# scroll-tech/zkevm-circuits

Measured on NVIDIA H100. Metric: SuperCircuit-shaped k=20 create_proof seconds (halo2 KZG/SHPLONK, Blake2b transcript), lower is better.
Workload: dtype u256 (8x u32 Montgomery limbs, BN254 Fr/Fq)

## Files before the change

zkevm-circuits_b200/csrc/common.cuh:

```cuda
#pragma once
#include <cuda_runtime.h>
#include <stdint.h>
#include <stdio.h>
#include <map>
#include <string>
#include <vector>
#include <array>
#include "../../include/zkb200.h"
#include "ff.cuh"
#include "g1.cuh"

namespace zkb {

void set_error(const char *fmt, ...);

#define ZKB_CUDA(expr)                                                                                   \
    do {                                                                                                 \
        cudaError_t _e = (expr);                                                                         \
        if (_e != cudaSuccess) {                                                                         \
            zkb::set_error("%s:%d %s -> %s", __FILE__, __LINE__, #expr, cudaGetErrorString(_e));         \
            return _e == cudaErrorMemoryAllocation ? ZKB_ERR_ALLOC : ZKB_ERR_CUDA;                       \
        }                                                                                                \
    } while (0)

#define ZKB_TRY(expr)                    \
    do {                                 \
        int32_t _r = (expr);             \
        if (_r != ZKB_OK) return _r;     \
    } while (0)

#define ZKB_ARG(cond)                                                            \
    do {                                                                         \
        if (!(cond)) {                                                           \
            zkb::set_error("%s:%d invalid argument: %s", __FILE__, __LINE__, #cond); \
            return ZKB_ERR_ARG;                                                  \
        }                                                                        \
    } while (0)

struct NttPlan {
    uint32_t log_n = 0;
    int npass = 0;
    int bits[3] = {0, 0, 0};
    Fr *tw_lo = nullptr;
    Fr *tw_hi = nullptr;
    Fr *loc[3] = {nullptr, nullptr, nullptr};
    Fr *tw_b[2] = {nullptr, nullptr};
    Fr *tw_b_scaled = nullptr;
    Fr scaled_key;
    bool has_scaled = false;
};

struct DeviceBuffer {
    void *ptr = nullptr;
    size_t bytes = 0;
};

}

struct zkb_ctx {
    int device = 0;
    cudaStream_t stream = nullptr;
    cudaStream_t copy_stream = nullptr;
    int sm_count = 132;
    size_t mem_bytes = 0;
    void *nccl_comm = nullptr;
    int rank = 0, nranks = 1;
    void *win_local = nullptr;
    size_t win_bytes = 0;
    void *win_peers[16] = {nullptr};
    std::map<std::array<uint64_t, 6>, void *> shard_tw;
    uint64_t launches = 0;
    bool prof_on = false;
    struct ProfPair { cudaEvent_t a, b; int cls; };
    std::vector<ProfPair> prof_pending;
    std::vector<cudaEvent_t> prof_free;
    double prof_ms[8] = {};
    uint64_t prof_count[8] = {};
    bool ntt_ready = false;
    uint64_t msm_last_adds = 0;
    uint32_t msm_last_levels = 0;
    std::map<std::array<uint64_t, 5>, zkb::NttPlan> ntt_plans;
    zkb::DeviceBuffer scratch[14];
    std::multimap<size_t, void *> block_cache;
    size_t block_cache_bytes = 0;
    void *pinned = nullptr;
    size_t pinned_bytes = 0;
};

struct zkb_srs {
    zkb_ctx *ctx = nullptr;
    uint32_t k = 0;
    uint64_t n = 0;
    zkb::G1Affine *g = nullptr, *g_lagrange = nullptr;
    zkb::G1Affine *g_shift = nullptr, *g_lagrange_shift = nullptr;
    std::vector<std::pair<void *, size_t>> blocks;
};

namespace zkb {
int32_t scratch_get(zkb_ctx *ctx, int slot, size_t bytes, void **out);
int32_t block_alloc(zkb_ctx *ctx, size_t bytes, void **out, size_t *got);
void block_free(zkb_ctx *ctx, void *p, size_t bytes);
inline cudaStream_t pick_stream(zkb_ctx *ctx, void *stream) { return stream ? (cudaStream_t)stream : ctx->stream; }
enum ProfClass { PROF_NTT = 0, PROF_MSM_ACC = 1, PROF_EXPR = 2, PROF_OTHER = 3, PROF_CHECK_GATES = 4, PROF_CHECK_LOOKUPS = 5,
                 PROF_CHECK_COPIES = 6, PROF_CHECK_EXTRACT = 7, PROF_CLASSES = 8 };
struct ProfScope {
    zkb_ctx *ctx;
    cudaStream_t st;
    cudaEvent_t a = nullptr, b = nullptr;
    int cls;
    ProfScope(zkb_ctx *c, int cl, cudaStream_t s) : ctx(c), st(s), cls(cl) {
        if (!ctx->prof_on) return;
        auto get = [&]() { cudaEvent_t e = nullptr; if (!ctx->prof_free.empty()) { e = ctx->prof_free.back(); ctx->prof_free.pop_back(); } else cudaEventCreate(&e); return e; };
        a = get(); b = get();
        cudaEventRecord(a, st);
    }
    ~ProfScope() {
        if (!a) return;
        cudaEventRecord(b, st);
        ctx->prof_pending.push_back({a, b, cls});
    }
};

Fr host_root_of_unity(uint32_t k);
Fr host_zeta();
int32_t ntt_fr_device(zkb_ctx *ctx, const Fr *src, Fr *dst, uint32_t log_n, const Fr &omega, const Fr *scale_host, int coset_zeta,
                      const Fr *d_in_scale, cudaStream_t st);
int32_t ntt_fr_batch_device(zkb_ctx *ctx, const Fr *const *h_src, Fr *const *h_dst, uint32_t count, uint32_t log_n,
                            const Fr &omega, const Fr *scale_host, int coset_zeta, const Fr *d_in_scale, cudaStream_t st);
struct NttPeerRoute {
    const Fr *out_tw;
    bool routed;
    uint32_t log_blk, rank;
    int nranks;
    Fr *peers[16];
};
int32_t ntt_fr_batch_device_ex(zkb_ctx *ctx, const Fr *const *h_src, Fr *const *h_dst, uint32_t count, uint32_t log_n, const Fr &omega,
                               const Fr *scale_host, int coset_zeta, const Fr *d_in_scale, const NttPeerRoute *route, cudaStream_t st);
int32_t msm_g1_device(zkb_ctx *ctx, const Fr *scalars, const G1Affine *bases, uint64_t n, G1Affine *out_affine_host, cudaStream_t st);
uint32_t msm_max_batch(uint64_t n);
uint32_t msm_shift_copies(uint64_t n);
int32_t msm_build_shifted_bases(zkb_ctx *ctx, const G1Affine *bases, uint64_t n, G1Affine *out, cudaStream_t st);
int32_t msm_g1_batch_device_ex(zkb_ctx *ctx, const Fr *const *d_scalar_cols, uint32_t batch, const G1Affine *bases, uint64_t n,
                               G1Affine *out_affine_host, bool shifted, cudaStream_t st);
int32_t msm_g1_batch_device(zkb_ctx *ctx, const Fr *const *d_scalar_cols, uint32_t batch, const G1Affine *bases, uint64_t n,
                            G1Affine *out_affine_host, cudaStream_t st);
int32_t srs_create(zkb_ctx *ctx, uint32_t k, const G1Affine *g, bool g_on_device, const G1Affine *g_lagrange, bool gl_on_device, zkb_srs **out);
int32_t srs_commit_many(zkb_srs *s, int basis, const Fr *const *cols, uint32_t count, uint64_t len, G1Affine *out_host, cudaStream_t st);
int32_t fr_powers_device(zkb_ctx *ctx, const Fr &base, uint64_t n, Fr *out, cudaStream_t st);
int32_t poly_eval_device(zkb_ctx *ctx, const Fr *const *d_polys, uint32_t num, uint64_t n, const Fr &x, Fr *out_host, cudaStream_t st);
int32_t prefix_product_device(zkb_ctx *ctx, const Fr *in, uint64_t n, const Fr &init, Fr *out, cudaStream_t st);
int32_t prefix_sum_device(zkb_ctx *ctx, const Fr *in, uint64_t n, const Fr &init, Fr *out, cudaStream_t st);
int32_t kate_division_device(zkb_ctx *ctx, const Fr *a, uint64_t n, const Fr &u, Fr *q, cudaStream_t st);
int32_t lincomb_device(zkb_ctx *ctx, const Fr *const *d_polys, const Fr *d_coefs, uint32_t num, uint64_t n, Fr *out, bool accumulate, cudaStream_t st);
int32_t batch_invert_device(zkb_ctx *ctx, const Fr *a, Fr *out, uint64_t n, cudaStream_t st);
int32_t comm_allreduce_u64(zkb_ctx *ctx, void *dev_buf, size_t count, cudaStream_t st);
int32_t comm_allgather(zkb_ctx *ctx, const void *send, void *recv, size_t bytes_per_rank, cudaStream_t st);
int32_t comm_alltoall(zkb_ctx *ctx, const void *send, void *recv, size_t bytes_per_block, cudaStream_t st);
int32_t comm_barrier(zkb_ctx *ctx, cudaStream_t st);
int32_t comm_window(zkb_ctx *ctx, size_t bytes, cudaStream_t st);

struct DevPool {
    zkb_ctx *ctx = nullptr;
    std::vector<std::pair<void *, size_t>> ptrs;
    ~DevPool() {
        if (!ctx) return;
        cudaStreamSynchronize(ctx->stream);
        for (auto &p : ptrs) block_free(ctx, p.first, p.second);
    }
    int32_t alloc(size_t bytes, void **out) {
        size_t got = 0;
        ZKB_TRY(block_alloc(ctx, bytes ? bytes : 32, out, &got));
        ptrs.push_back({*out, got});
        return ZKB_OK;
    }
    int32_t fr(uint64_t n, Fr **out) { return alloc(n * sizeof(Fr), (void **)out); }
};

enum ScratchSlot { SCR_NTT = 0, SCR_MSM_A = 1, SCR_MSM_B = 2, SCR_MSM_C = 3, SCR_HOSTIO_A = 4, SCR_HOSTIO_B = 5, SCR_MISC = 6, SCR_MISC2 = 7, SCR_MSM_TBL = 8, SCR_COMM = 9, SCR_NTT_DESC = 10, SCR_MSM_D = 11, SCR_COMM_FLAG = 12, SCR_SHARD = 13 };
}
```

zkevm-circuits_b200/csrc/msm.cu:

```cuda
#include "common.cuh"
#include <string.h>
#include <algorithm>

namespace zkb {

struct MsmCfg {
    uint32_t c;
    uint32_t windows;
    uint32_t half;
    uint32_t seg_log;
    uint32_t shifted;
    uint32_t n32;
};

static MsmCfg choose_cfg(uint64_t n) {
    uint32_t lg = 0;
    while ((1ull << (lg + 1)) <= n) ++lg;
    int c = (int)lg - 4;
    if (c < 3) c = 3;
    if (c > 20) c = 20;
    MsmCfg m;
    m.c = (uint32_t)c;
    m.windows = (255 + m.c - 1) / m.c;
    m.half = 1u << (m.c - 1);
    m.seg_log = 0;
    m.shifted = 0;
    m.n32 = 0;
    return m;
}

__device__ __forceinline__ uint32_t raw_window(const uint32_t s[8], uint32_t bit, uint32_t c) {
    const uint32_t limb = bit >> 5, off = bit & 31;
    uint64_t v = s[limb];
    if (limb + 1 < 8) v |= (uint64_t)s[limb + 1] << 32;
    return (uint32_t)(v >> off) & ((1u << c) - 1);
}

template <int MODE>
__global__ void msm_digits_kernel(const Fr *const *__restrict__ scalar_cols, uint64_t n, MsmCfg m, uint32_t *__restrict__ counts,
                                  uint32_t *__restrict__ cursors, uint32_t *__restrict__ sorted) {
    const uint64_t i = blockIdx.x * (uint64_t)blockDim.x + threadIdx.x;
    if (i >= n) return;
    const uint32_t col_base = blockIdx.y * (m.shifted ? m.half : m.windows * m.half);
    const Fr s = fp_to_canonical(fp_load(scalar_cols[blockIdx.y] + i));
    uint32_t carry = 0;
    for (uint32_t w = 0; w < m.windows; ++w) {
        const uint32_t bit = w * m.c;
        uint32_t d = (bit < 256 ? raw_window(s.l, bit, m.c) : 0) + carry;
        uint32_t neg = 0;
        if (d > m.half) { d = (1u << m.c) - d; neg = 1; carry = 1; }
        else carry = 0;
        if (d != 0) {
            const uint32_t b = col_base + (m.shifted ? 0u : w * m.half) + (d - 1);
            if (MODE == 0) atomicAdd(&counts[b], 1u);
            else {
                const uint32_t pos = atomicAdd(&cursors[b], 1u);
                sorted[pos] = ((uint32_t)i + (m.shifted ? w * m.n32 : 0u)) | (neg << 31);
            }
        }
    }
}

constexpr int SCAN_T = 512, SCAN_PER = 4, SCAN_BLK = SCAN_T * SCAN_PER;

__device__ __forceinline__ uint32_t block_exclusive_scan(uint32_t v, uint32_t *total, uint32_t *sm ) {
    const uint32_t lane = threadIdx.x & 31, wid = threadIdx.x >> 5;
    uint32_t x = v;
#pragma unroll
    for (int o = 1; o < 32; o <<= 1) {
        uint32_t y = __shfl_up_sync(0xffffffffu, x, o);
        if (lane >= o) x += y;
    }
    if (lane == 31) sm[wid] = x;
    __syncthreads();
    if (wid == 0) {
        uint32_t t = lane < (blockDim.x >> 5) ? sm[lane] : 0;
#pragma unroll
        for (int o = 1; o < 32; o <<= 1) {
            uint32_t y = __shfl_up_sync(0xffffffffu, t, o);
            if (lane >= o) t += y;
        }
        sm[lane] = t;
    }
    __syncthreads();
    const uint32_t base = wid ? sm[wid - 1] : 0;
    *total = sm[(blockDim.x >> 5) - 1];
    return base + x - v;
}

__global__ void scan_blocks_kernel(const uint32_t *__restrict__ in, uint32_t *__restrict__ out, uint32_t *__restrict__ block_sums, uint64_t n) {
    __shared__ uint32_t sm[32];
    const uint64_t base = (uint64_t)blockIdx.x * SCAN_BLK + (uint64_t)threadIdx.x * SCAN_PER;
    uint32_t v[SCAN_PER], sum = 0;
#pragma unroll
    for (int k = 0; k < SCAN_PER; ++k) { v[k] = base + k < n ? in[base + k] : 0; sum += v[k]; }
    uint32_t total;
    uint32_t ex = block_exclusive_scan(sum, &total, sm);
#pragma unroll
    for (int k = 0; k < SCAN_PER; ++k) { if (base + k < n) out[base + k] = ex; ex += v[k]; }
    if (threadIdx.x == 0) block_sums[blockIdx.x] = total;
}
__global__ void scan_sums_kernel(uint32_t *__restrict__ block_sums, uint32_t nblocks, uint32_t *__restrict__ grand_total) {
    __shared__ uint32_t sm[32];
    uint32_t running = 0;
    for (uint32_t s = 0; s < nblocks; s += SCAN_T) {
        const uint32_t idx = s + threadIdx.x;
        const uint32_t v = idx < nblocks ? block_sums[idx] : 0;
        uint32_t total;
        const uint32_t ex = block_exclusive_scan(v, &total, sm);
        if (idx < nblocks) block_sums[idx] = running + ex;
        running += total;
        __syncthreads();
    }
    if (threadIdx.x == 0 && grand_total) *grand_total = running;
}
__global__ void scan_add_kernel(uint32_t *__restrict__ out, const uint32_t *__restrict__ block_sums, uint64_t n) {
    const uint64_t base = (uint64_t)blockIdx.x * SCAN_BLK + (uint64_t)threadIdx.x * SCAN_PER;
    const uint32_t add = block_sums[blockIdx.x];
#pragma unroll
    for (int k = 0; k < SCAN_PER; ++k)
        if (base + k < n) out[base + k] += add;
}

struct MsmState;
__global__ void scan_blocks_gated_kernel(const uint32_t *__restrict__ in, uint32_t *const outs0, uint32_t *const outs1, const uint32_t *st_words,
                                         uint32_t *__restrict__ block_sums, uint64_t n) {
    if (st_words[0] <= 1) return;
    uint32_t *out = st_words[1] ? outs0 : outs1;
    __shared__ uint32_t sm[32];
    const uint64_t base = (uint64_t)blockIdx.x * SCAN_BLK + (uint64_t)threadIdx.x * SCAN_PER;
    uint32_t v[SCAN_PER], sum = 0;
#pragma unroll
    for (int k = 0; k < SCAN_PER; ++k) { v[k] = base + k < n ? in[base + k] : 0; sum += v[k]; }
    uint32_t total;
    uint32_t ex = block_exclusive_scan(sum, &total, sm);
#pragma unroll
    for (int k = 0; k < SCAN_PER; ++k) { if (base + k < n) out[base + k] = ex; ex += v[k]; }
    if (threadIdx.x == 0) block_sums[blockIdx.x] = total;
}
__global__ void scan_sums_gated_kernel(uint32_t *__restrict__ block_sums, uint32_t nblocks, uint32_t *const outs0, uint32_t *const outs1,
                                       const uint32_t *st_words, uint64_t n) {
    if (st_words[0] <= 1) return;
    uint32_t *out = st_words[1] ? outs0 : outs1;
    __shared__ uint32_t sm[32];
    uint32_t running = 0;
    for (uint32_t s = 0; s < nblocks; s += SCAN_T) {
        const uint32_t idx = s + threadIdx.x;
        const uint32_t v = idx < nblocks ? block_sums[idx] : 0;
        uint32_t total;
        const uint32_t ex = block_exclusive_scan(v, &total, sm);
        if (idx < nblocks) block_sums[idx] = running + ex;
        running += total;
        __syncthreads();
    }
    if (threadIdx.x == 0) out[n] = running;
}
__global__ void scan_add_gated_kernel(uint32_t *const outs0, uint32_t *const outs1, const uint32_t *st_words, const uint32_t *__restrict__ block_sums,
                                      uint64_t n) {
    if (st_words[0] <= 1) return;
    uint32_t *out = st_words[1] ? outs0 : outs1;
    const uint64_t base = (uint64_t)blockIdx.x * SCAN_BLK + (uint64_t)threadIdx.x * SCAN_PER;
    const uint32_t add = block_sums[blockIdx.x];
#pragma unroll
    for (int k = 0; k < SCAN_PER; ++k)
        if (base + k < n) out[base + k] += add;
}

static void exclusive_scan_u32(zkb_ctx *ctx, const uint32_t *in, uint32_t *out, uint64_t n, uint32_t *tmp, cudaStream_t st) {
    const uint32_t nblocks = (uint32_t)((n + SCAN_BLK - 1) / SCAN_BLK);
    scan_blocks_kernel<<<nblocks, SCAN_T, 0, st>>>(in, out, tmp, n);
    scan_sums_kernel<<<1, SCAN_T, 0, st>>>(tmp, nblocks, out + n);
    scan_add_kernel<<<nblocks, SCAN_T, 0, st>>>(out, tmp, n);
    ctx->launches += 3;
}

constexpr uint32_t ACC_CH = 64;
constexpr uint32_t CHUNK = 32;

struct MsmState {
    uint32_t maxlen;
    uint32_t cur;
    uint32_t levels_run;
    uint32_t pad;
    uint64_t extra_adds;
};

__global__ void chunk_count_kernel(const uint32_t *__restrict__ seg_off, uint32_t nseg, uint32_t *__restrict__ tcount, MsmState *st) {
    const uint32_t b = blockIdx.x * blockDim.x + threadIdx.x;
    uint32_t cnt = 0;
    if (b < nseg) {
        const uint32_t lo = seg_off[b], hi = seg_off[b + 1];
        cnt = hi > lo ? (hi - 1) / CHUNK - lo / CHUNK + 1 : 0;
        tcount[b] = cnt;
    }
    for (int o = 16; o > 0; o >>= 1) {
        const uint32_t y = __shfl_down_sync(0xffffffffu, cnt, o);
        cnt = y > cnt ? y : cnt;
    }
    if ((threadIdx.x & 31) == 0 && cnt > 1) atomicMax(&st->maxlen, cnt);
}
__device__ __forceinline__ uint32_t find_segment(const uint32_t *__restrict__ toff, uint32_t nseg, uint32_t t) {
    uint32_t lo = 0, hi = nseg;
    while (hi - lo > 1) {
        const uint32_t mid = (lo + hi) >> 1;
        if (toff[mid] <= t) lo = mid; else hi = mid;
    }
    return lo;
}
__global__ void __launch_bounds__(128) msm_acc_chunk_kernel(const G1Affine *__restrict__ bases, const uint32_t *__restrict__ seg_off,
                                                           const uint32_t *__restrict__ sorted, const uint32_t *__restrict__ toff,
                                                           uint32_t nseg, G1Xyzz *__restrict__ part) {
    const uint32_t total = seg_off[nseg];
    const uint32_t t = blockIdx.x * blockDim.x + threadIdx.x;
    const uint32_t beg = t * CHUNK;
    if (beg >= total) return;
    const uint32_t end = beg + CHUNK < total ? beg + CHUNK : total;
    uint32_t b = find_segment(seg_off, nseg, beg);
    uint32_t b_first = seg_off[b], next = seg_off[b + 1];
    G1Xyzz acc = G1Xyzz::identity();
    uint32_t e = sorted[beg];
    G1Affine p = g1_load_affine(bases + (e & 0x7fffffffu));
    for (uint32_t k = beg; k < end; ++k) {
        if (k == next) {
            g1_store_xyzz(part + toff[b] + (t - b_first / CHUNK), acc);
            acc = G1Xyzz::identity();
            do { ++b; next = seg_off[b + 1]; } while (next <= k);
            b_first = seg_off[b];
        }
        const uint32_t e_cur = e;
        const G1Affine p_cur = p;
        if (k + 1 < end) {
            e = sorted[k + 1];
            p = g1_load_affine(bases + (e & 0x7fffffffu));
        }
        g1_add_mixed(acc, (e_cur >> 31) ? g1_neg(p_cur) : p_cur);
    }
    g1_store_xyzz(part + toff[b] + (t - b_first / CHUNK), acc);
}

struct LevelBufs {
    uint32_t *toff[2];
    G1Xyzz *part[2];
    uint32_t *tcount;
    MsmState *st;
};
__global__ void level_task_count_kernel(LevelBufs L, uint32_t nseg) {
    if (L.st->maxlen <= 1) return;
    const uint32_t *seg_off = L.toff[L.st->cur];
    const uint32_t b = blockIdx.x * blockDim.x + threadIdx.x;
    if (b >= nseg) return;
    const uint32_t len = seg_off[b + 1] - seg_off[b];
    L.tcount[b] = (len + ACC_CH - 1) / ACC_CH;
}
__global__ void __launch_bounds__(128) msm_acc_levelN_kernel(LevelBufs L, uint32_t nseg) {
    if (L.st->maxlen <= 1) return;
    const uint32_t cur = L.st->cur;
    const uint32_t *__restrict__ seg_off = L.toff[cur];
    const uint32_t *__restrict__ toff = L.toff[cur ^ 1];
    const G1Xyzz *__restrict__ in = L.part[cur];
    G1Xyzz *__restrict__ part = L.part[cur ^ 1];
    const uint32_t ntasks = toff[nseg];
    for (uint32_t t = blockIdx.x * blockDim.x + threadIdx.x; t < ntasks; t += gridDim.x * blockDim.x) {
        const uint32_t b = find_segment(toff, nseg, t);
        const uint32_t beg = seg_off[b] + (t - toff[b]) * ACC_CH;
        const uint32_t lim = seg_off[b + 1];
        const uint32_t end = beg + ACC_CH < lim ? beg + ACC_CH : lim;
        G1Xyzz acc = g1_load_xyzz(in + beg);
        for (uint32_t k = beg + 1; k < end; ++k) g1_add(acc, g1_load_xyzz(in + k));
        g1_store_xyzz(part + t, acc);
    }
}
__global__ void level_advance_kernel(LevelBufs L, uint32_t nseg) {
    MsmState *st = L.st;
    if (st->maxlen <= 1) return;
    const uint32_t cur = st->cur;
    st->extra_adds += L.toff[cur][nseg];
    st->maxlen = (st->maxlen + ACC_CH - 1) / ACC_CH;
    st->cur = cur ^ 1;
    st->levels_run++;
}
__global__ void msm_gather_buckets_kernel(LevelBufs L, uint32_t nseg, G1Xyzz *__restrict__ buckets) {
    const uint32_t b = blockIdx.x * blockDim.x + threadIdx.x;
    if (b >= nseg) return;
    const uint32_t cur = L.st->cur;
    const uint32_t *seg_off = L.toff[cur];
    const uint32_t beg = seg_off[b], end = seg_off[b + 1];
    g1_store_xyzz(buckets + b, end > beg ? g1_load_xyzz(L.part[cur] + beg) : G1Xyzz::identity());
}

__global__ void __launch_bounds__(128) msm_wsum_level_kernel(const G1Xyzz *__restrict__ in, uint32_t count, uint32_t log_l, uint32_t windows,
                                                            G1Xyzz *__restrict__ acc_out, G1Xyzz *__restrict__ run_out) {
    const uint32_t L = 1u << log_l;
    const uint32_t segs = (count + L - 1) >> log_l;
    const uint32_t t = blockIdx.x * blockDim.x + threadIdx.x;
    if (t >= windows * segs) return;
    const uint32_t w = t / segs, s = t % segs;
    const uint32_t base = s << log_l;
    const uint32_t len = count - base < L ? count - base : L;
    const G1Xyzz *p = in + (size_t)w * count + base;
    G1Xyzz running = G1Xyzz::identity(), acc = G1Xyzz::identity();
    for (int j = (int)len - 1; j >= 1; --j) {
        g1_add(running, g1_load_xyzz(p + j));
        g1_add(acc, running);
    }
    g1_add(running, g1_load_xyzz(p));
    g1_store_xyzz(acc_out + t, acc);
    g1_store_xyzz(run_out + t, running);
}
__global__ void __launch_bounds__(256) msm_window_sum_kernel(const G1Xyzz *__restrict__ partials, G1Xyzz *__restrict__ window_sums, uint32_t segs) {
    extern __shared__ uint4 sm4[];
    G1Xyzz *sm = reinterpret_cast<G1Xyzz *>(sm4);
    const uint32_t w = blockIdx.x;
    G1Xyzz acc = G1Xyzz::identity();
    for (uint32_t s = threadIdx.x; s < segs; s += blockDim.x) g1_add(acc, g1_load_xyzz(partials + (size_t)w * segs + s));
    sm[threadIdx.x] = acc;
    __syncthreads();
    for (uint32_t o = blockDim.x >> 1; o > 0; o >>= 1) {
        if (threadIdx.x < o) {
            G1Xyzz a = sm[threadIdx.x];
            g1_add(a, sm[threadIdx.x + o]);
            sm[threadIdx.x] = a;
        }
        __syncthreads();
    }
    if (threadIdx.x == 0) g1_store_xyzz(window_sums + w, sm[0]);
}
__global__ void msm_window_combine_kernel(const G1Xyzz *__restrict__ level_sums, const G1Xyzz *__restrict__ all_sum, uint32_t nlevels,
                                          uint32_t log_l, uint32_t windows, G1Xyzz *__restrict__ out) {
    const uint32_t w = blockIdx.x * blockDim.x + threadIdx.x;
    if (w >= windows) return;
    G1Xyzz r = g1_load_xyzz(level_sums + (size_t)(nlevels - 1) * windows + w);
    for (int lv = (int)nlevels - 2; lv >= 0; --lv) {
        for (uint32_t d = 0; d < log_l; ++d) r = g1_dbl(r);
        g1_add(r, g1_load_xyzz(level_sums + (size_t)lv * windows + w));
    }
    g1_add(r, g1_load_xyzz(all_sum + w));
    g1_store_xyzz(out + w, r);
}

__global__ void __launch_bounds__(128) msm_shift_bases_kernel(const G1Affine *__restrict__ in, G1Affine *__restrict__ out, uint64_t n, uint32_t c) {
    const uint64_t i = blockIdx.x * (uint64_t)blockDim.x + threadIdx.x;
    if (i >= n) return;
    G1Xyzz p = G1Xyzz::from_affine(g1_load_affine(in + i));
    for (uint32_t k = 0; k < c; ++k) p = g1_dbl(p);
    g1_store_affine(out + i, g1_to_affine(p));
}

__global__ void __launch_bounds__(128) fixed_base_mul_kernel(G1Affine base, const Fr *__restrict__ scalars, uint64_t n, G1Affine *__restrict__ out) {
    const uint64_t i = blockIdx.x * (uint64_t)blockDim.x + threadIdx.x;
    if (i >= n) return;
    const Fr s = fp_to_canonical(fp_load(scalars + i));
    G1Xyzz acc = G1Xyzz::identity();
    for (int bit = 253; bit >= 0; --bit) {
        acc = g1_dbl(acc);
        if ((s.l[bit >> 5] >> (bit & 31)) & 1) g1_add_mixed(acc, base);
    }
    g1_store_affine(out + i, g1_to_affine(acc));
}

static size_t align_up(size_t v, size_t a) { return (v + a - 1) / a * a; }

uint32_t msm_shift_window_bits(uint64_t n);
uint32_t msm_max_batch(uint64_t n) {
    if (n == 0) return 64;
    const MsmCfg m = choose_cfg(n);
    uint64_t b = (1ull << 28) / (n * m.windows);
    const uint32_t cs = msm_shift_window_bits(n);
    if (cs) {
        const uint64_t bb = (1ull << 31) / ((1ull << (cs - 1)) * 3 * sizeof(G1Xyzz));
        if (bb < b) b = bb;
    }
    if (b < 1) b = 1;
    if (b > 64) b = 64;
    return (uint32_t)b;
}

uint32_t msm_shift_window_bits(uint64_t n) {
    uint32_t lg = 0;
    while ((1ull << (lg + 1)) <= n) ++lg;
    if (lg < 10 || lg > 22) return 0;
    return lg > 20 ? 20 : lg;
}
uint32_t msm_shift_copies(uint64_t n) {
    const uint32_t c = msm_shift_window_bits(n);
    return c ? (255 + c - 1) / c : 0;
}
int32_t msm_build_shifted_bases(zkb_ctx *ctx, const G1Affine *bases, uint64_t n, G1Affine *out, cudaStream_t st) {
    const uint32_t c = msm_shift_window_bits(n), copies = msm_shift_copies(n);
    ZKB_ARG(c != 0);
    ZKB_CUDA(cudaMemcpyAsync(out, bases, n * sizeof(G1Affine), cudaMemcpyDeviceToDevice, st));
    for (uint32_t w = 1; w < copies; ++w) {
        msm_shift_bases_kernel<<<(unsigned)((n + 127) / 128), 128, 0, st>>>(out + (size_t)(w - 1) * n, out + (size_t)w * n, n, c);
        ctx->launches++;
    }
    ZKB_CUDA(cudaGetLastError());
    return ZKB_OK;
}

int32_t msm_g1_batch_device_ex(zkb_ctx *ctx, const Fr *const *d_scalar_cols, uint32_t batch, const G1Affine *bases, uint64_t n,
                               G1Affine *out_affine_host, bool shifted, cudaStream_t st);

int32_t msm_g1_batch_device(zkb_ctx *ctx, const Fr *const *d_scalar_cols, uint32_t batch, const G1Affine *bases, uint64_t n,
                            G1Affine *out_affine_host, cudaStream_t st) {
    return msm_g1_batch_device_ex(ctx, d_scalar_cols, batch, bases, n, out_affine_host, false, st);
}

int32_t msm_g1_batch_device_ex(zkb_ctx *ctx, const Fr *const *d_scalar_cols, uint32_t batch, const G1Affine *bases, uint64_t n,
                               G1Affine *out_affine_host, bool shifted, cudaStream_t st) {
    ZKB_ARG(n < (1ull << 31) && batch >= 1);
    if (n == 0) {
        memset(out_affine_host, 0, sizeof(G1Affine) * batch);
        ctx->msm_last_adds = 0;
        return ZKB_OK;
    }
    MsmCfg m = choose_cfg(n);
    if (shifted) {
        m.c = msm_shift_window_bits(n);
        ZKB_ARG(m.c != 0);
        m.windows = (255 + m.c - 1) / m.c;
        m.half = 1u << (m.c - 1);
        m.shifted = 1;
        m.n32 = (uint32_t)n;
        ZKB_ARG((uint64_t)m.windows * n < (1ull << 31));
    }
    const uint32_t windows1 = m.windows;
    const uint32_t rwin1 = shifted ? 1 : windows1;
    const uint32_t nbuckets = batch * rwin1 * m.half;
    const uint64_t pairs = n * windows1 * batch;
    ZKB_ARG(pairs < (1ull << 32) && (uint64_t)batch * rwin1 * m.half < (1ull << 31));
    uint32_t log_l = 5;
    while (log_l > 3 && (uint64_t)batch * rwin1 * (m.half >> log_l) < 32768) --log_l;

    const size_t cnt_bytes = align_up((size_t)(nbuckets + 2) * 4, 256);
    const size_t tmp_bytes = align_up(((size_t)nbuckets / SCAN_BLK + 2) * 4, 256);
    uint8_t *A = nullptr, *B = nullptr, *C = nullptr;
    ZKB_TRY(scratch_get(ctx, SCR_MSM_A, 6 * cnt_bytes + tmp_bytes + 256, (void **)&A));
    ZKB_TRY(scratch_get(ctx, SCR_MSM_B, pairs * 4, (void **)&B));
    uint32_t *counts = (uint32_t *)A, *offsets = (uint32_t *)(A + cnt_bytes), *cursors = (uint32_t *)(A + 2 * cnt_bytes);
    uint32_t *tcount = (uint32_t *)(A + 3 * cnt_bytes), *toff[2] = {(uint32_t *)(A + 4 * cnt_bytes), (uint32_t *)(A + 5 * cnt_bytes)};
    uint32_t *scan_tmp = (uint32_t *)(A + 6 * cnt_bytes);
    MsmState *d_state = (MsmState *)(A + 6 * cnt_bytes + tmp_bytes);
    uint32_t *sorted = (uint32_t *)B;

    const uint32_t half = m.half;
    const uint32_t wred = rwin1 * batch;
    uint32_t nlevels = 0, cnt = half;
    size_t level_entries = 0;
    while (cnt > 1) { cnt = (cnt + (1u << log_l) - 1) >> log_l; level_entries += 2ull * cnt * wred; nlevels++; }
    if (nlevels == 0) { nlevels = 1; level_entries = 2ull * wred; }
    const size_t part0_n = (size_t)((pairs + CHUNK - 1) / CHUNK) + nbuckets + 1;
    const size_t part1_n = part0_n / ACC_CH + nbuckets + 1;
    ZKB_ARG(part0_n < (1ull << 32));
    const size_t c_entries = part0_n + part1_n + nbuckets + level_entries + (size_t)nlevels * wred + 2ull * wred;
    ZKB_TRY(scratch_get(ctx, SCR_MSM_C, c_entries * sizeof(G1Xyzz), (void **)&C));
    G1Xyzz *part[2] = {(G1Xyzz *)C, (G1Xyzz *)C + part0_n};
    G1Xyzz *buckets = part[1] + part1_n, *lvl = buckets + nbuckets, *lvl_sums = lvl + level_entries, *all_sum = lvl_sums + (size_t)nlevels * wred,
           *wres = all_sum + wred;

    ZKB_CUDA(cudaMemsetAsync(counts, 0, cnt_bytes, st));
    ZKB_CUDA(cudaMemsetAsync(d_state, 0, sizeof(MsmState), st));
    const unsigned tb = 256, bb = (nbuckets + 255) / 256;
    const dim3 gb((unsigned)((n + tb - 1) / tb), batch);
    msm_digits_kernel<0><<<gb, tb, 0, st>>>(d_scalar_cols, n, m, counts, nullptr, nullptr);
    exclusive_scan_u32(ctx, counts, offsets, nbuckets, scan_tmp, st);
    ZKB_CUDA(cudaMemcpyAsync(cursors, offsets, (size_t)nbuckets * 4, cudaMemcpyDeviceToDevice, st));
    msm_digits_kernel<1><<<gb, tb, 0, st>>>(d_scalar_cols, n, m, nullptr, cursors, sorted);
    m.windows = wred;
    chunk_count_kernel<<<bb, 256, 0, st>>>(offsets, nbuckets, tcount, d_state);
    exclusive_scan_u32(ctx, tcount, toff[0], nbuckets, scan_tmp, st);
    {
        const uint64_t max_chunks = (pairs + CHUNK - 1) / CHUNK;
        ProfScope ps_(ctx, PROF_MSM_ACC, st);
        msm_acc_chunk_kernel<<<(unsigned)((max_chunks + 127) / 128), 128, 0, st>>>(bases, offsets, sorted, toff[0], nbuckets, part[0]);
    }
    ctx->launches += 4;
    LevelBufs L;
    L.toff[0] = toff[0]; L.toff[1] = toff[1];
    L.part[0] = part[0]; L.part[1] = part[1];
    L.tcount = tcount;
    L.st = d_state;
    {
        uint64_t bound = (n * (shifted ? windows1 : 1) + CHUNK - 1) / CHUNK + 1;
        const uint32_t nscan = (uint32_t)(((uint64_t)nbuckets + SCAN_BLK - 1) / SCAN_BLK);
        const uint32_t *stw = (const uint32_t *)d_state;
        const unsigned lv_blocks = (unsigned)std::min<uint64_t>((part0_n / ACC_CH + nbuckets + 127) / 128, (uint64_t)ctx->sm_count * 32);
        while (bound > 1) {
            level_task_count_kernel<<<bb, 256, 0, st>>>(L, nbuckets);
            scan_blocks_gated_kernel<<<nscan, SCAN_T, 0, st>>>(tcount, toff[0], toff[1], stw, scan_tmp, nbuckets);
            scan_sums_gated_kernel<<<1, SCAN_T, 0, st>>>(scan_tmp, nscan, toff[0], toff[1], stw, nbuckets);
            scan_add_gated_kernel<<<nscan, SCAN_T, 0, st>>>(toff[0], toff[1], stw, scan_tmp, nbuckets);
            msm_acc_levelN_kernel<<<lv_blocks, 128, 0, st>>>(L, nbuckets);
            level_advance_kernel<<<1, 1, 0, st>>>(L, nbuckets);
            ctx->launches += 6;
            bound = (bound + ACC_CH - 1) / ACC_CH;
        }
    }
    msm_gather_buckets_kernel<<<bb, 256, 0, st>>>(L, nbuckets, buckets);
    ctx->launches++;

    {
        const G1Xyzz *in = buckets;
        uint32_t count = half;
        G1Xyzz *p = lvl;
        for (uint32_t lv = 0; lv < nlevels; ++lv) {
            const uint32_t segs = (count + (1u << log_l) - 1) >> log_l;
            G1Xyzz *acc_out = p, *run_out = p + (size_t)segs * m.windows;
            msm_wsum_level_kernel<<<(m.windows * segs + 127) / 128, 128, 0, st>>>(in, count, log_l, m.windows, acc_out, run_out);
            uint32_t wt = 32;
            while (wt < segs && wt < 256) wt <<= 1;
            msm_window_sum_kernel<<<m.windows, wt, wt * sizeof(G1Xyzz), st>>>(acc_out, lvl_sums + (size_t)lv * m.windows, segs);
            ctx->launches += 2;
            in = run_out;
            count = segs;
            p += 2ull * segs * m.windows;
            if (lv + 1 == nlevels) {
                ZKB_CUDA(cudaMemcpyAsync(all_sum, run_out, (size_t)m.windows * sizeof(G1Xyzz), cudaMemcpyDeviceToDevice, st));
            }
        }
        msm_window_combine_kernel<<<(m.windows + 31) / 32, 32, 0, st>>>(lvl_sums, all_sum, nlevels, log_l, m.windows, wres);
        ctx->launches++;
    }
    ZKB_CUDA(cudaGetLastError());

    std::vector<G1Xyzz> h(m.windows);
    MsmState h_state;
    uint32_t total_pairs = 0;
    ZKB_CUDA(cudaMemcpyAsync(h.data(), wres, m.windows * sizeof(G1Xyzz), cudaMemcpyDeviceToHost, st));
    ZKB_CUDA(cudaMemcpyAsync(&h_state, d_state, sizeof(MsmState), cudaMemcpyDeviceToHost, st));
    ZKB_CUDA(cudaMemcpyAsync(&total_pairs, offsets + nbuckets, 4, cudaMemcpyDeviceToHost, st));
    ZKB_CUDA(cudaStreamSynchronize(st));
    for (uint32_t col = 0; col < batch; ++col) {
        const G1Xyzz *hw = h.data() + (size_t)col * rwin1;
        G1Xyzz acc = hw[rwin1 - 1];
        for (int w = (int)rwin1 - 2; w >= 0; --w) {
            for (uint32_t k = 0; k < m.c; ++k) acc = g1_dbl(acc);
            g1_add(acc, hw[w]);
        }
        out_affine_host[col] = g1_to_affine(acc);
    }
    ctx->msm_last_adds = (uint64_t)total_pairs + h_state.extra_adds + 2ull * nbuckets;
    ctx->msm_last_levels = h_state.levels_run;
    return ZKB_OK;
}

int32_t msm_g1_device(zkb_ctx *ctx, const Fr *scalars, const G1Affine *bases, uint64_t n, G1Affine *out_affine_host, cudaStream_t st) {
    if (n == 0) {
        memset(out_affine_host, 0, sizeof(G1Affine));
        ctx->msm_last_adds = 0;
        return ZKB_OK;
    }
    const Fr **d_tbl = nullptr;
    ZKB_TRY(scratch_get(ctx, SCR_MSM_TBL, 64 * sizeof(Fr *), (void **)&d_tbl));
    ZKB_CUDA(cudaMemcpyAsync(d_tbl, &scalars, sizeof(Fr *), cudaMemcpyHostToDevice, st));
    return msm_g1_batch_device(ctx, d_tbl, 1, bases, n, out_affine_host, st);
}

}
using namespace zkb;

static void emit_outputs(const G1Affine &r, uint64_t out_affine[8], uint64_t *out_jacobian, uint8_t *out_compressed) {
    memcpy(out_affine, &r, 64);
    if (out_jacobian) {
        memcpy(out_jacobian, &r, 64);
        Fq z = r.is_identity() ? Fq::zero() : Fq::one();
        memcpy(out_jacobian + 8, &z, 32);
    }
    if (out_compressed) g1_compress(r, out_compressed);
}

extern "C" int32_t zkb_msm_g1_dev(zkb_ctx *ctx, const uint64_t *scalars_dev, const uint64_t *bases_dev, uint64_t n, uint64_t out_affine[8],
                                  uint64_t *out_jacobian, uint8_t *out_compressed, void *stream) {
    ZKB_ARG(ctx && out_affine && (n == 0 || (scalars_dev && bases_dev)));
    ZKB_CUDA(cudaSetDevice(ctx->device));
    G1Affine r;
    ZKB_TRY(msm_g1_device(ctx, (const Fr *)scalars_dev, (const G1Affine *)bases_dev, n, &r, pick_stream(ctx, stream)));
    emit_outputs(r, out_affine, out_jacobian, out_compressed);
    return ZKB_OK;
}

extern "C" int32_t zkb_msm_g1_host(zkb_ctx *ctx, const uint64_t *scalars_host, const uint64_t *bases_host, uint64_t n, uint64_t out_affine[8],
                                   uint64_t *out_jacobian, uint8_t *out_compressed) {
    ZKB_ARG(ctx && out_affine && (n == 0 || (scalars_host && bases_host)));
    ZKB_CUDA(cudaSetDevice(ctx->device));
    void *ds = nullptr, *db = nullptr;
    if (n) {
        ZKB_TRY(scratch_get(ctx, SCR_HOSTIO_A, n * 32, &ds));
        ZKB_TRY(scratch_get(ctx, SCR_HOSTIO_B, n * 64, &db));
        ZKB_CUDA(cudaMemcpyAsync(ds, scalars_host, n * 32, cudaMemcpyHostToDevice, ctx->stream));
        ZKB_CUDA(cudaMemcpyAsync(db, bases_host, n * 64, cudaMemcpyHostToDevice, ctx->stream));
    }
    return zkb_msm_g1_dev(ctx, (const uint64_t *)ds, (const uint64_t *)db, n, out_affine, out_jacobian, out_compressed, ctx->stream);
}

extern "C" int32_t zkb_msm_g1_batch_dev(zkb_ctx *ctx, const uint64_t *const *scalar_cols_dev, uint32_t batch, const uint64_t *bases_dev, uint64_t n,
                                        uint64_t *out_affine, void *stream) {
    ZKB_ARG(ctx && scalar_cols_dev && bases_dev && out_affine && batch >= 1);
    ZKB_CUDA(cudaSetDevice(ctx->device));
    cudaStream_t st = pick_stream(ctx, stream);
    const uint32_t maxb = msm_max_batch(n);
    for (uint32_t done = 0; done < batch; done += maxb) {
        const uint32_t cur = batch - done < maxb ? batch - done : maxb;
        const Fr **d_tbl = nullptr;
        ZKB_TRY(scratch_get(ctx, SCR_MSM_TBL, 64 * sizeof(Fr *), (void **)&d_tbl));
        ZKB_CUDA(cudaMemcpyAsync(d_tbl, scalar_cols_dev + done, cur * sizeof(Fr *), cudaMemcpyHostToDevice, st));
        ZKB_TRY(msm_g1_batch_device(ctx, d_tbl, cur, (const G1Affine *)bases_dev, n, (G1Affine *)out_affine + done, st));
    }
    return ZKB_OK;
}

extern "C" int32_t zkb_g1_fixed_base_mul_dev(zkb_ctx *ctx, const uint64_t base_affine_host[8], const uint64_t *scalars_dev, uint64_t n,
                                             uint64_t *out_affine_dev, void *stream) {
    ZKB_ARG(ctx && base_affine_host && scalars_dev && out_affine_dev);
    if (n == 0) return ZKB_OK;
    G1Affine base;
    memcpy(&base, base_affine_host, 64);
    fixed_base_mul_kernel<<<(unsigned)((n + 127) / 128), 128, 0, pick_stream(ctx, stream)>>>(base, (const Fr *)scalars_dev, n, (G1Affine *)out_affine_dev);
    ctx->launches++;
    ZKB_CUDA(cudaGetLastError());
    return ZKB_OK;
}
```

Measured before the change: 1.565.

## Prefetch MSM bucket bases via cp.async shared-memory ring in accumulation kernel

Rewrites the MSM chunk accumulation kernel so each thread stages the next four affine bases into a per-thread shared-memory ring with cp.async. It also loads sorted indices four at a time as uint4 and packs sign bits into a mask. The aim is to hide global-memory latency on the gathered base loads behind the mixed-add arithmetic. The cost is 40KB of static shared memory per block, which may reduce occupancy. It also adds profiling scopes for the MSM sort and tail phases and widens the profiler class arrays.

```diff
diff --git a/zkevm-circuits_b200/csrc/common.cuh b/zkevm-circuits_b200/csrc/common.cuh
--- a/zkevm-circuits_b200/csrc/common.cuh
+++ b/zkevm-circuits_b200/csrc/common.cuh
@@ -50,6 +50,9 @@
     bool has_scaled = false;
 };
 
+enum ProfClass { PROF_NTT = 0, PROF_MSM_ACC = 1, PROF_EXPR = 2, PROF_OTHER = 3, PROF_CHECK_GATES = 4, PROF_CHECK_LOOKUPS = 5,
+                 PROF_CHECK_COPIES = 6, PROF_CHECK_EXTRACT = 7, PROF_MSM_SORT = 8, PROF_MSM_TAIL = 9, PROF_CLASSES = 10 };
+
 struct DeviceBuffer {
     void *ptr = nullptr;
     size_t bytes = 0;
@@ -74,8 +77,8 @@
     struct ProfPair { cudaEvent_t a, b; int cls; };
     std::vector<ProfPair> prof_pending;
     std::vector<cudaEvent_t> prof_free;
-    double prof_ms[8] = {};
-    uint64_t prof_count[8] = {};
+    double prof_ms[zkb::PROF_CLASSES] = {};
+    uint64_t prof_count[zkb::PROF_CLASSES] = {};
     bool ntt_ready = false;
     uint64_t msm_last_adds = 0;
     uint32_t msm_last_levels = 0;
@@ -101,8 +104,6 @@
 int32_t block_alloc(zkb_ctx *ctx, size_t bytes, void **out, size_t *got);
 void block_free(zkb_ctx *ctx, void *p, size_t bytes);
 inline cudaStream_t pick_stream(zkb_ctx *ctx, void *stream) { return stream ? (cudaStream_t)stream : ctx->stream; }
-enum ProfClass { PROF_NTT = 0, PROF_MSM_ACC = 1, PROF_EXPR = 2, PROF_OTHER = 3, PROF_CHECK_GATES = 4, PROF_CHECK_LOOKUPS = 5,
-                 PROF_CHECK_COPIES = 6, PROF_CHECK_EXTRACT = 7, PROF_CLASSES = 8 };
 struct ProfScope {
     zkb_ctx *ctx;
     cudaStream_t st;
diff --git a/zkevm-circuits_b200/csrc/msm.cu b/zkevm-circuits_b200/csrc/msm.cu
--- a/zkevm-circuits_b200/csrc/msm.cu
+++ b/zkevm-circuits_b200/csrc/msm.cu
@@ -207,33 +207,90 @@
     }
     return lo;
 }
-__global__ void __launch_bounds__(128) msm_acc_chunk_kernel(const G1Affine *__restrict__ bases, const uint32_t *__restrict__ seg_off,
-                                                           const uint32_t *__restrict__ sorted, const uint32_t *__restrict__ toff,
-                                                           uint32_t nseg, G1Xyzz *__restrict__ part) {
+constexpr uint32_t ACC_T = 128;
+constexpr uint32_t ACC_AHEAD = 4;
+constexpr uint32_t ACC_RING = ACC_AHEAD + 1;
+static_assert(CHUNK <= 32, "the chunk's sign bits live in one 32-bit mask");
+
+__device__ __forceinline__ uint4 load_idx4(const uint32_t *__restrict__ sorted, uint32_t pos, uint32_t total) {
+    if (pos + 4 <= total) return __ldg(reinterpret_cast<const uint4 *>(sorted + pos));
+    uint4 v = make_uint4(0, 0, 0, 0);
+    if (pos + 0 < total) v.x = sorted[pos + 0];
+    if (pos + 1 < total) v.y = sorted[pos + 1];
+    if (pos + 2 < total) v.z = sorted[pos + 2];
+    return v;
+}
+__device__ __forceinline__ uint32_t quad_lane(const uint4 &v, uint32_t i) { return i == 0 ? v.x : i == 1 ? v.y : i == 2 ? v.z : v.w; }
+__device__ __forceinline__ void stage_base(uint4 *ring, uint32_t slot, const G1Affine *__restrict__ bases, uint32_t e) {
+    const char *src = reinterpret_cast<const char *>(bases + (e & 0x7fffffffu));
+#pragma unroll
+    for (uint32_t q = 0; q < 4; ++q) {
+        const uint32_t dst = (uint32_t)__cvta_generic_to_shared(ring + (slot * 4 + q) * ACC_T + threadIdx.x);
+        asm volatile("cp.async.cg.shared.global [%0], [%1], 16;" ::"r"(dst), "l"(src + 16 * q) : "memory");
+    }
+}
+__device__ __forceinline__ G1Affine read_base(const uint4 *ring, uint32_t slot) {
+    G1Affine p;
+    uint4 v[4];
+#pragma unroll
+    for (uint32_t q = 0; q < 4; ++q) v[q] = ring[(slot * 4 + q) * ACC_T + threadIdx.x];
+#pragma unroll
+    for (uint32_t q = 0; q < 2; ++q) {
+        p.x.l[4 * q + 0] = v[q].x; p.x.l[4 * q + 1] = v[q].y; p.x.l[4 * q + 2] = v[q].z; p.x.l[4 * q + 3] = v[q].w;
+        p.y.l[4 * q + 0] = v[q + 2].x; p.y.l[4 * q + 1] = v[q + 2].y; p.y.l[4 * q + 2] = v[q + 2].z; p.y.l[4 * q + 3] = v[q + 2].w;
+    }
+    return p;
+}
+
+__global__ void __launch_bounds__(ACC_T) msm_acc_chunk_kernel(const G1Affine *__restrict__ bases, const uint32_t *__restrict__ seg_off,
+                                                             const uint32_t *__restrict__ sorted, const uint32_t *__restrict__ toff,
+                                                             uint32_t nseg, G1Xyzz *__restrict__ part) {
+    __shared__ uint4 ring[ACC_RING * 4 * ACC_T];
     const uint32_t total = seg_off[nseg];
     const uint32_t t = blockIdx.x * blockDim.x + threadIdx.x;
     const uint32_t beg = t * CHUNK;
     if (beg >= total) return;
-    const uint32_t end = beg + CHUNK < total ? beg + CHUNK : total;
+    const uint32_t len = total - beg < CHUNK ? total - beg : CHUNK;
     uint32_t b = find_segment(seg_off, nseg, beg);
     uint32_t b_first = seg_off[b], next = seg_off[b + 1];
+    uint4 quad = load_idx4(sorted, beg, total);
+    uint4 quad_next = load_idx4(sorted, beg + 4, total);
+    uint32_t neg = 0;
+#pragma unroll
+    for (uint32_t j = 0; j < ACC_AHEAD; ++j) {
+        if (j < len) {
+            const uint32_t e = quad_lane(quad, j);
+            neg |= (e >> 31) << j;
+            stage_base(ring, j, bases, e);
+        }
+        asm volatile("cp.async.commit_group;" ::: "memory");
+    }
     G1Xyzz acc = G1Xyzz::identity();
-    uint32_t e = sorted[beg];
-    G1Affine p = g1_load_affine(bases + (e & 0x7fffffffu));
-    for (uint32_t k = beg; k < end; ++k) {
+    uint32_t slot = 0;
+    for (uint32_t j = 0; j < len; ++j) {
+        const uint32_t k = beg + j;
         if (k == next) {
             g1_store_xyzz(part + toff[b] + (t - b_first / CHUNK), acc);
             acc = G1Xyzz::identity();
             do { ++b; next = seg_off[b + 1]; } while (next <= k);
             b_first = seg_off[b];
         }
-        const uint32_t e_cur = e;
-        const G1Affine p_cur = p;
-        if (k + 1 < end) {
-            e = sorted[k + 1];
-            p = g1_load_affine(bases + (e & 0x7fffffffu));
-        }
-        g1_add_mixed(acc, (e_cur >> 31) ? g1_neg(p_cur) : p_cur);
+        const uint32_t i = j & 3;
+        if (i == 0) {
+            quad = quad_next;
+            if (j + 8 < len) quad_next = load_idx4(sorted, k + 8, total);
+        }
+        const uint32_t ahead = j + ACC_AHEAD;
+        if (ahead < len) {
+            const uint32_t e = quad_lane(quad, i);
+            neg |= (e >> 31) << ahead;
+            stage_base(ring, slot == 0 ? ACC_RING - 1 : slot - 1, bases, e);
+        }
+        asm volatile("cp.async.commit_group;" ::: "memory");
+        asm volatile("cp.async.wait_group %0;" ::"n"(ACC_AHEAD) : "memory");
+        const G1Affine p = read_base(ring, slot);
+        g1_add_mixed(acc, (neg >> j) & 1 ? g1_neg(p) : p);
+        slot = slot + 1 == ACC_RING ? 0 : slot + 1;
     }
     g1_store_xyzz(part + toff[b] + (t - b_first / CHUNK), acc);
 }
@@ -461,17 +518,23 @@
     ZKB_CUDA(cudaMemsetAsync(d_state, 0, sizeof(MsmState), st));
     const unsigned tb = 256, bb = (nbuckets + 255) / 256;
     const dim3 gb((unsigned)((n + tb - 1) / tb), batch);
-    msm_digits_kernel<0><<<gb, tb, 0, st>>>(d_scalar_cols, n, m, counts, nullptr, nullptr);
-    exclusive_scan_u32(ctx, counts, offsets, nbuckets, scan_tmp, st);
-    ZKB_CUDA(cudaMemcpyAsync(cursors, offsets, (size_t)nbuckets * 4, cudaMemcpyDeviceToDevice, st));
-    msm_digits_kernel<1><<<gb, tb, 0, st>>>(d_scalar_cols, n, m, nullptr, cursors, sorted);
+    {
+        ProfScope ps_(ctx, PROF_MSM_SORT, st);
+        msm_digits_kernel<0><<<gb, tb, 0, st>>>(d_scalar_cols, n, m, counts, nullptr, nullptr);
+        exclusive_scan_u32(ctx, counts, offsets, nbuckets, scan_tmp, st);
+        ZKB_CUDA(cudaMemcpyAsync(cursors, offsets, (size_t)nbuckets * 4, cudaMemcpyDeviceToDevice, st));
+        msm_digits_kernel<1><<<gb, tb, 0, st>>>(d_scalar_cols, n, m, nullptr, cursors, sorted);
+    }
     m.windows = wred;
-    chunk_count_kernel<<<bb, 256, 0, st>>>(offsets, nbuckets, tcount, d_state);
-    exclusive_scan_u32(ctx, tcount, toff[0], nbuckets, scan_tmp, st);
+    {
+        ProfScope ps_(ctx, PROF_MSM_TAIL, st);
+        chunk_count_kernel<<<bb, 256, 0, st>>>(offsets, nbuckets, tcount, d_state);
+        exclusive_scan_u32(ctx, tcount, toff[0], nbuckets, scan_tmp, st);
+    }
     {
         const uint64_t max_chunks = (pairs + CHUNK - 1) / CHUNK;
         ProfScope ps_(ctx, PROF_MSM_ACC, st);
-        msm_acc_chunk_kernel<<<(unsigned)((max_chunks + 127) / 128), 128, 0, st>>>(bases, offsets, sorted, toff[0], nbuckets, part[0]);
+        msm_acc_chunk_kernel<<<(unsigned)((max_chunks + ACC_T - 1) / ACC_T), ACC_T, 0, st>>>(bases, offsets, sorted, toff[0], nbuckets, part[0]);
     }
     ctx->launches += 4;
     LevelBufs L;
@@ -480,6 +543,7 @@
     L.tcount = tcount;
     L.st = d_state;
     {
+        ProfScope ps_(ctx, PROF_MSM_TAIL, st);
         uint64_t bound = (n * (shifted ? windows1 : 1) + CHUNK - 1) / CHUNK + 1;
         const uint32_t nscan = (uint32_t)(((uint64_t)nbuckets + SCAN_BLK - 1) / SCAN_BLK);
         const uint32_t *stw = (const uint32_t *)d_state;
@@ -494,11 +558,12 @@
             ctx->launches += 6;
             bound = (bound + ACC_CH - 1) / ACC_CH;
         }
-    }
-    msm_gather_buckets_kernel<<<bb, 256, 0, st>>>(L, nbuckets, buckets);
-    ctx->launches++;
+        msm_gather_buckets_kernel<<<bb, 256, 0, st>>>(L, nbuckets, buckets);
+        ctx->launches++;
+    }
 
     {
+        ProfScope ps_(ctx, PROF_MSM_TAIL, st);
         const G1Xyzz *in = buckets;
         uint32_t count = half;
         G1Xyzz *p = lvl;
```

Measured after the change: 1.547 (median of 6 runs). -1.1%, faster.
